# Zhen-Dong/HAWQ

Measured on NVIDIA H100. Metric: images/sec ResNet-50 W8A8 & W4A4 @batch128, 1/2/4/8xH100; % int-TC roofline, higher is better.
Workload: dtype int8

## Files before the change

### hawq_b200/csrc/api.cu

```cuda
#include <cmath>
#include <cstdarg>
#include <cstdio>
#include <cstring>

#include <cstdlib>

#include "conv_igemm.cuh"
#include "elementwise.cuh"
#include "stem.cuh"

using namespace hawq;

struct hawq_handle {
  int device;
  int sm_count;
  int32_t* status;
};

static thread_local char g_err[512] = "";
static long long g_kernel_count[8] = {0, 0, 0, 0, 0, 0, 0, 0};

static int fail(int code, const char* fmt, ...) {
  va_list ap;
  va_start(ap, fmt);
  vsnprintf(g_err, sizeof(g_err), fmt, ap);
  va_end(ap);
  return code;
}

#define CUDA_TRY(expr)                                                                         \
  do {                                                                                         \
    cudaError_t _e = (expr);                                                                   \
    if (_e != cudaSuccess) return fail(HAWQ_ERR_CUDA, "%s: %s", #expr, cudaGetErrorString(_e)); \
  } while (0)

static int launch_check(const char* what) {
  cudaError_t e = cudaGetLastError();
  if (e != cudaSuccess) return fail(HAWQ_ERR_CUDA, "%s launch: %s", what, cudaGetErrorString(e));
  return HAWQ_OK;
}

static int grid_for(long long work_items, int sm_count) {
  long long blocks = (work_items + 255) / 256;
  const long long cap = (long long)sm_count * 16;
  if (blocks > cap) blocks = cap;
  if (blocks < 1) blocks = 1;
  return (int)blocks;
}

template <int BN, bool A4, int FAM, bool DUAL>
static int set_conv_attr1() {
  CUDA_TRY(cudaFuncSetAttribute(conv_igemm_kernel<BN, A4, FAM, DUAL>, cudaFuncAttributeMaxDynamicSharedMemorySize,
                                ConvSmem<BN, A4, DUAL>::TOTAL));
  CUDA_TRY(cudaFuncSetAttribute(conv_igemm_kernel<BN, A4, FAM, DUAL>, cudaFuncAttributePreferredSharedMemoryCarveout,
                                cudaSharedmemCarveoutMaxShared));
  return HAWQ_OK;
}
template <int BN, bool A4>
static int set_conv_attr() {
  int rc;
  if ((rc = set_conv_attr1<BN, A4, FAM_REQUANT, false>()) || (rc = set_conv_attr1<BN, A4, FAM_RESIDUAL, false>()) ||
      (rc = set_conv_attr1<BN, A4, FAM_STORE, false>()))
    return rc;
  return HAWQ_OK;
}

static dim3 conv_grid(long long M, int Cout, int BN) { return dim3((unsigned)((M + CONV_BM - 1) / CONV_BM * (Cout / BN)), 1, 1); }

template <int BN, bool A4>
static void launch_conv(const ConvParams& p, cudaStream_t s) {
  const int smem = ConvSmem<BN, A4, false>::TOTAL;
  const dim3 grid = conv_grid(p.M, p.Cout, BN);
  if (p.mode == HAWQ_EPI_REQUANT) conv_igemm_kernel<BN, A4, FAM_REQUANT, false><<<grid, CONV_THREADS, smem, s>>>(p);
  else if (p.mode == HAWQ_EPI_RESIDUAL) conv_igemm_kernel<BN, A4, FAM_RESIDUAL, false><<<grid, CONV_THREADS, smem, s>>>(p);
  else conv_igemm_kernel<BN, A4, FAM_STORE, false><<<grid, CONV_THREADS, smem, s>>>(p);
}
template <bool A4>
static void launch_conv_dual(const ConvParams& p, cudaStream_t s) {
  conv_igemm_kernel<64, A4, FAM_RESIDUAL, true><<<conv_grid(p.M, p.Cout, 64), CONV_THREADS, ConvSmem<64, A4, true>::TOTAL, s>>>(p);
}

extern "C" {

int hawq_abi_version(void) { return HAWQ_ABI_VERSION; }
const char* hawq_last_error(void) { return g_err; }

int hawq_create(int device, hawq_handle** out) {
  if (!out) return fail(HAWQ_ERR_BAD_ARG, "hawq_create: out is null");
  CUDA_TRY(cudaSetDevice(device));
  cudaDeviceProp prop;
  CUDA_TRY(cudaGetDeviceProperties(&prop, device));
  if (prop.major != 9 || prop.minor != 0)
    return fail(HAWQ_ERR_UNSUPPORTED, "hawq_create: device sm_%d%d is not Hopper sm_90 (the library is built for sm_90a)", prop.major, prop.minor);
  hawq_handle* h = new hawq_handle();
  h->device = device;
  h->sm_count = prop.multiProcessorCount;
  h->status = nullptr;
  CUDA_TRY(cudaMalloc(&h->status, sizeof(int32_t)));
  CUDA_TRY(cudaMemset(h->status, 0, sizeof(int32_t)));
  int rc;
  CUDA_TRY(cudaFuncSetAttribute(linear_dp4a_kernel, cudaFuncAttributeMaxDynamicSharedMemorySize, linear_smem_bytes(LIN_MAX_K)));
  if ((rc = set_conv_attr<128, false>()) || (rc = set_conv_attr<64, false>()) || (rc = set_conv_attr<128, true>()) ||
      (rc = set_conv_attr<64, true>()) || (rc = set_conv_attr1<64, false, FAM_RESIDUAL, true>()) ||
      (rc = set_conv_attr1<64, true, FAM_RESIDUAL, true>()))
    return rc;
  *out = h;
  return HAWQ_OK;
}

int hawq_destroy(hawq_handle* h) {
  if (!h) return HAWQ_OK;
  cudaFree(h->status);
  delete h;
  return HAWQ_OK;
}

int hawq_sm_count(const hawq_handle* h) { return h ? h->sm_count : 0; }

int hawq_reset_status(hawq_handle* h, void* stream) {
  if (!h) return fail(HAWQ_ERR_BAD_ARG, "null handle");
  CUDA_TRY(cudaMemsetAsync(h->status, 0, sizeof(int32_t), (cudaStream_t)stream));
  return HAWQ_OK;
}

int hawq_get_status(hawq_handle* h, void* stream, int32_t* host_flags) {
  if (!h || !host_flags) return fail(HAWQ_ERR_BAD_ARG, "null argument");
  CUDA_TRY(cudaMemcpyAsync(host_flags, h->status, sizeof(int32_t), cudaMemcpyDeviceToHost, (cudaStream_t)stream));
  CUDA_TRY(cudaStreamSynchronize((cudaStream_t)stream));
  return HAWQ_OK;
}

int hawq_copy_status(hawq_handle* h, int32_t* dst, void* stream) {
  if (!h || !dst) return fail(HAWQ_ERR_BAD_ARG, "null argument");
  CUDA_TRY(cudaMemcpyAsync(dst, h->status, sizeof(int32_t), cudaMemcpyDeviceToDevice, (cudaStream_t)stream));
  return HAWQ_OK;
}

static void set_bias_window(ConvParams& p, int a_bits) {
// ... 56 lines not shown
        if (!res_chan) return fail(HAWQ_ERR_BAD_ARG, "hawq_conv2d: res_kind 1 needs res_chan");
      } else if (ep->res_kind == 0) {
        if (ep->res_bits != 16 && ep->res_bits != 32) return fail(HAWQ_ERR_BAD_ARG, "hawq_conv2d: res_bits must be 16/32");
        int rc = check_me(ep->res_m, ep->res_e, "hawq_conv2d residual");
        if (rc) return rc;
      } else return fail(HAWQ_ERR_BAD_ARG, "hawq_conv2d: res_kind must be 0/1");
      if (ep->y_bits != 0 && ep->y_bits != 16 && ep->y_bits != 32) return fail(HAWQ_ERR_BAD_ARG, "hawq_conv2d: y_bits must be 0/16/32");
      if (ep->y_bits == 16 && !ep->relu) return fail(HAWQ_ERR_BAD_ARG, "hawq_conv2d: uint16 residual stream requires relu");
      if (ep->y_bits && !out) return fail(HAWQ_ERR_BAD_ARG, "hawq_conv2d: y_bits set but out is null");
      if (ep->low_bits != 0 && ep->low_bits != 4 && ep->low_bits != 8) return fail(HAWQ_ERR_BAD_ARG, "hawq_conv2d: low_bits must be 0/4/8");
      if (ep->low_bits) {
        if (!out_low) return fail(HAWQ_ERR_BAD_ARG, "hawq_conv2d: low_bits set but out_low is null");
        int rc = check_me(ep->low_m, ep->low_e, "hawq_conv2d low-bit copy");
        if (rc) return rc;
      }
      if (!ep->y_bits && !ep->low_bits) return fail(HAWQ_ERR_BAD_ARG, "hawq_conv2d: RESIDUAL with no output");
      break;
    case HAWQ_EPI_RAW_I32:
      if (!out) return fail(HAWQ_ERR_BAD_ARG, "hawq_conv2d: RAW_I32 needs out");
      break;
    case HAWQ_EPI_DEQUANT_F32:
      if (!out || !fscale) return fail(HAWQ_ERR_BAD_ARG, "hawq_conv2d: DEQUANT_F32 needs out and fscale");
      if (ep->cout_store < 1 || ep->cout_store > d->Cout) return fail(HAWQ_ERR_BAD_ARG, "hawq_conv2d: bad cout_store");
      break;
    default:
      return fail(HAWQ_ERR_BAD_ARG, "hawq_conv2d: unknown epilogue mode %d", ep->mode);
  }

  const bool bn128 = (d->Cout % 128 == 0);
  if ((M + CONV_BM - 1) / CONV_BM * (d->Cout / (bn128 ? 128 : 64)) > 0x7fffffffll)
    return fail(HAWQ_ERR_UNSUPPORTED, "hawq_conv2d: more than 2^31 - 1 output tiles");
  ++g_kernel_count[0];
  cudaStream_t s = (cudaStream_t)stream;
  if (d->a_bits == 8) {
    if (bn128) launch_conv<128, false>(p, s);
    else launch_conv<64, false>(p, s);
  } else {
    if (bn128) launch_conv<128, true>(p, s);
    else launch_conv<64, true>(p, s);
  }
  return launch_check("conv_igemm");
}

int hawq_conv2d_dual(hawq_handle* h, const hawq_conv_desc* d, const hawq_epilogue_desc* ep, const void* x, const int8_t* w,
                     const hawq_chan* chan, const hawq_conv_desc* d2, const void* x2, const int8_t* w2, const hawq_chan* chan2,
                     void* out, void* out_low, void* stream) {
  if (!h || !d || !ep || !x || !w || !chan || !d2 || !x2 || !w2 || !chan2 || !out) return fail(HAWQ_ERR_BAD_ARG, "hawq_conv2d_dual: null argument");
  if (d->kh != 1 || d->kw != 1 || d->stride != 1 || d->pad != 0 || d2->kh != 1 || d2->kw != 1 || d2->pad != 0 || d2->stride < 1)
    return fail(HAWQ_ERR_UNSUPPORTED, "hawq_conv2d_dual: both convolutions must be 1x1 without padding (main stride 1)");
  if (d->N < 1 || d->H < 1 || d->W < 1 || d2->H < 1 || d2->W < 1) return fail(HAWQ_ERR_BAD_ARG, "hawq_conv2d_dual: bad geometry");
  if ((d->a_bits != 8 && d->a_bits != 4) || d2->a_bits != d->a_bits) return fail(HAWQ_ERR_UNSUPPORTED, "hawq_conv2d_dual: a_bits must be equal and 4 or 8");
  if (d->Cin % 64 || d2->Cin % 64 || d->Cout % 64 || d2->Cout != d->Cout) return fail(HAWQ_ERR_UNSUPPORTED, "hawq_conv2d_dual: channel counts must be multiples of 64 and Cout equal");
  if (d2->N != d->N || (d2->H - 1) / d2->stride + 1 != d->H || (d2->W - 1) / d2->stride + 1 != d->W)
    return fail(HAWQ_ERR_BAD_ARG, "hawq_conv2d_dual: the two convolutions have different output grids");
  if (d->w_layout != 1 || d2->w_layout != 1) return fail(HAWQ_ERR_UNSUPPORTED, "hawq_conv2d_dual: weights must carry the re-tiled copy (w_layout 1)");
  if (ep->mode != HAWQ_EPI_RESIDUAL || !ep->relu || ep->y_bits != 16) return fail(HAWQ_ERR_UNSUPPORTED, "hawq_conv2d_dual: RESIDUAL + relu + uint16 stream only");
  if (ep->low_bits != 0 && ep->low_bits != 4 && ep->low_bits != 8) return fail(HAWQ_ERR_BAD_ARG, "hawq_conv2d_dual: low_bits must be 0/4/8");
  if (ep->low_bits) {
    if (!out_low) return fail(HAWQ_ERR_BAD_ARG, "hawq_conv2d_dual: low_bits set but out_low is null");
    int rc = check_me(ep->low_m, ep->low_e, "hawq_conv2d_dual low-bit copy");
    if (rc) return rc;
    if (!dyadic_is_fast(ep->low_m, ep->low_e)) return fail(HAWQ_ERR_UNSUPPORTED, "hawq_conv2d_dual: low-bit ratio outside the fast range");
  }
  const bool ratios_one = (ep->flags & HAWQ_EP_RATIOS_LE_ONE) != 0;
  const bool ratios_wide = !ratios_one && (ep->flags & HAWQ_EP_RATIOS_LE_2P20) != 0;
  if (!ratios_one && !ratios_wide) return fail(HAWQ_ERR_UNSUPPORTED, "hawq_conv2d_dual: needs a ratio-range promise (flags)");
// ... 244 lines not shown
```

### hawq_b200/csrc/conv_igemm.cuh

```cuda
#pragma once
#include <type_traits>

#include "common.cuh"
#include "wgmma.cuh"

namespace hawq {

struct ConvParams {
  const uint8_t* x;
  const int8_t* w;
  const hawq_chan* chan;
  const void* res;
  const hawq_chan* res_chan;
  const float* fscale;
  void* out;
  void* out_low;
  int32_t* status;
  int N, H, W, Cin, Cout, KH, KW, stride, pad, Ho, Wo, M, K;
  int cin_chunks;
  int x_pix_bytes;
  int mode, relu, out_bits, lo, hi;
  int res_kind, res_bits;
  uint32_t res_m;
  int res_e;
  int y_bits, low_bits;
  uint32_t low_m;
  int low_e, low_lo, low_hi;
  int cout_store;
  int scalar_over_one;
  int scalar_unchecked;
  int check_ovf;
  int bias_lo, bias_hi;
  const uint8_t* x2;
  const int8_t* w2;
  int H2, W2, stride2, cin_chunks2, x2_pix_bytes;
};

constexpr int CONV_BM = 128;
constexpr int CONV_STAGES = 4;
constexpr int CONV_THREADS = 256;

template <int BN, bool A4, bool DUAL>
struct ConvSmem {
  static constexpr int A_ROW = A4 ? 32 : 64;
  static constexpr int A_STAGE = CONV_BM * A_ROW;
  static constexpr int B_STAGE = BN * 64;
  static constexpr int PIPE = CONV_STAGES * (A_STAGE + B_STAGE);
  static constexpr int OUT_PITCH = BN + 16;
  static constexpr int OUT_STAGE = CONV_BM * OUT_PITCH;
  static constexpr int RES16 = CONV_BM * (BN * 2 + 16);
  static constexpr int RES32 = CONV_BM * (BN * 4 + 32);
  static constexpr int RES16_OFF = PIPE;
  static constexpr int RES32_OFF = DUAL ? PIPE : OUT_STAGE;
  static constexpr int Y_OFF = OUT_STAGE;
  static constexpr int MAIN = DUAL ? PIPE + RES32 : (PIPE + RES16 > RES32_OFF + RES32 ? PIPE + RES16 : RES32_OFF + RES32);
  static constexpr int CHAN_OFF = MAIN;
  static constexpr int M_OFF = CHAN_OFF + BN * (int)sizeof(hawq_chan);
  static constexpr int M1_OFF = M_OFF + BN * 8;
  static constexpr int RC_OFF = M1_OFF + BN * 8;
  static constexpr int CB_OFF = RC_OFF + BN * (int)sizeof(hawq_chan);
  static constexpr int TOTAL = CB_OFF + BN * 8;
  static_assert(OUT_STAGE <= PIPE && (!DUAL || Y_OFF + RES16 <= PIPE), "the epilogue staging tiles must fit in the freed ring");
  static_assert(2 * (TOTAL + 1024) <= 228 * 1024, "two CTAs per SM must fit in shared memory");
};

template <int ROW_BYTES>
__device__ __forceinline__ int swz(int row, int ch) {
  if constexpr (ROW_BYTES == 64) return row * 64 + ((ch ^ ((row >> 1) & 3)) << 4);
  else return row * 32 + ((ch ^ ((row >> 2) & 1)) << 4);
}

constexpr int FAM_REQUANT = 0, FAM_RESIDUAL = 1, FAM_STORE = 2;

template <bool CLAMPED>
struct RqFp64 {
  bool checked;
  bool ovf = false;
  static constexpr double kMagic = 6755399441055744.0;
  __device__ static double acc_bias(int32_t acc, double cb, int32_t) {
    const double d = __hiloint2double(0x43300000, acc ^ 0x80000000) - cb;
    return CLAMPED ? fmin(fmax(d, -2147483648.0), 2147483647.0) : d;
  }
  __device__ static double of_i32(int32_t v) {
    return __hiloint2double(0x43300000, v ^ 0x80000000) - 4503601774854144.0;
  }
  __device__ static double of_u16(uint32_t u) { return __hiloint2double(0x43300000, (int)u) - 4503599627370496.0; }
  __device__ int32_t term(double d, double M, uint32_t, int32_t, bool count) {
    const double t = __fma_rn(d, M, kMagic);
    if (checked && count) {
      const double q = t - kMagic;
      ovf |= q > 2147483647.0 || q < -2147483648.0;
    }
    return __double2loint(t);
  }
};
struct RqExact {
  bool checked;
  bool ovf = false;
  __device__ static int32_t acc_bias(int32_t acc, double, int32_t bias) { return sat_add(acc, bias); }
  __device__ static int32_t of_i32(int32_t v) { return v; }
  __device__ static int32_t of_u16(uint32_t u) { return (int32_t)u; }
  __device__ int32_t term(int32_t v, double, uint32_t m, int32_t e, bool count) {
    const long long q = rhe_requant64(v, m, e);
    if (checked && count) ovf |= q > 2147483647ll || q < -2147483648ll;
    return sat_i32(q);
  }
};

struct ConvGeom {
  const uint8_t* x;
  const int8_t* w;
  int H, W, stride, pad, KH, KW, cin_chunks, x_pix_bytes, K;
};

template <int BN, bool A4, int FAM, bool DUAL>
__global__ void __launch_bounds__(CONV_THREADS, 2) conv_igemm_kernel(const ConvParams p) {
  using S = ConvSmem<BN, A4, DUAL>;
  constexpr int BM = CONV_BM, STAGES = CONV_STAGES;
  constexpr int A_ROW = S::A_ROW;
  constexpr int A_CH = A_ROW / 16;
  constexpr int A_ROWS_PER_PASS = CONV_THREADS / A_CH;
  constexpr int A_PASSES = BM / A_ROWS_PER_PASS;
  constexpr int B_PASSES = BN / 64;
  constexpr int NT = BN / 8;
  constexpr int NACC = BN / 2;

  extern __shared__ __align__(1024) uint8_t smem[];
  uint8_t* sA = smem;
  uint8_t* sB = smem + STAGES * S::A_STAGE;
  hawq_chan* sChan = reinterpret_cast<hawq_chan*>(smem + S::CHAN_OFF);
  double* sM = reinterpret_cast<double*>(smem + S::M_OFF);
  double* sM1 = reinterpret_cast<double*>(smem + S::M1_OFF);
  hawq_chan* sResChan = reinterpret_cast<hawq_chan*>(smem + S::RC_OFF);
  double* sCb = reinterpret_cast<double*>(smem + S::CB_OFF);

  const int tid = threadIdx.x;
  const int lane = tid & 31, warp = tid >> 5;
  const int wg = warp >> 2;
  const int g = lane >> 2, t = lane & 3;
  const int nblk = p.Cout / BN;
  const int m0 = (int)(blockIdx.x / nblk) * BM;
  const int n0 = (int)(blockIdx.x % nblk) * BN;

  int over_one = p.scalar_over_one;
  int unchecked = p.scalar_unchecked;
  int bias_out = 0;
  if (tid < BN) {
    const hawq_chan c = p.chan[n0 + tid];
    sChan[tid] = c;
    sM[tid] = dyadic_to_double(c.m, c.e);
    sCb[tid] = 4503601774854144.0 - (double)c.bias;
    bias_out = c.bias < p.bias_lo || c.bias > p.bias_hi;
    over_one |= !dyadic_is_fast(c.m, c.e);
    unchecked |= !dyadic_is_wide(c.m, c.e);
    if (FAM == FAM_RESIDUAL && p.res_kind == 1) {
      const hawq_chan rc = p.res_chan[n0 + tid];
      sResChan[tid] = rc;
      sM1[tid] = dyadic_to_double(rc.m, rc.e);
      over_one |= !dyadic_is_fast(rc.m, rc.e);
      unchecked |= !dyadic_is_wide(rc.m, rc.e);
    }
  }
  const bool ratio_over_one = __syncthreads_or(over_one) != 0;
  const bool ratio_unchecked = __syncthreads_or(unchecked) != 0;
  const bool clamped = __syncthreads_or(bias_out) != 0;
  const bool fp64 = !ratio_over_one || (FAM == FAM_RESIDUAL && p.check_ovf && !ratio_unchecked);

  int32_t acc[NACC];

  const int res_es = (FAM == FAM_RESIDUAL) ? ((p.res_kind == 1 || p.res_bits == 32) ? 4 : 2) : 0;
  const int res_pitch = BN * res_es + 8 * res_es;
  uint8_t* sRes = smem + (res_es == 2 ? S::RES16_OFF : S::RES32_OFF);

  auto load_res = [&]() {
    if constexpr (FAM == FAM_RESIDUAL) {
      const int cpr = BN * res_es / 16;
      const uint8_t* gres = reinterpret_cast<const uint8_t*>(p.res);
      for (int id = tid; id < BM * cpr; id += CONV_THREADS) {
        const int row = id / cpr, j = id - row * cpr;
        const bool v = m0 + row < p.M;
        const uint8_t* src = v ? gres + ((size_t)(m0 + row) * p.Cout + n0) * res_es + j * 16 : gres;
        cp_async_16(smem_u32(sRes + row * res_pitch + j * 16), src, v ? 16 : 0);
      }
    }
  };
  const bool prefetch_res = !DUAL && res_es == 2;

  auto gemm = [&](const ConvGeom& gm, bool with_res) {
#pragma unroll
    for (int i = 0; i < NACC; ++i) acc[i] = 0;
    const int a_ch = tid % A_CH;
    int a_hi0[A_PASSES], a_wi0[A_PASSES], a_pix[A_PASSES];
    bool a_ok[A_PASSES];
#pragma unroll
    for (int i = 0; i < A_PASSES; ++i) {
      const int row = tid / A_CH + i * A_ROWS_PER_PASS;
      const int m = m0 + row;
      a_ok[i] = m < p.M;
      const int mm = a_ok[i] ? m : 0;
// ... 48 lines not shown
      cp_async_commit();

      const int stage = kt % STAGES;
      const uint32_t a_base = smem_u32(sA + stage * S::A_STAGE);
      const uint32_t b_base = smem_u32(sB + stage * S::B_STAGE);
#pragma unroll
      for (int ks = 0; ks < 2; ++ks) {
        const uint64_t bdesc = wgmma_desc_sw64(b_base + ks * 32);
        if constexpr (!A4) {
          wgmma_fence();
          wgmma_ss<BN>(acc, wgmma_desc_sw64(a_base + wg * 64 * A_ROW + ks * 32), bdesc);
        } else {
          uint32_t r0, r1;
          const int row = warp * 16 + (lane & 7) + ((lane >> 3) & 1) * 8;
          ldmatrix_x2(r0, r1, a_base + swz<32>(row, ks));
          const uint32_t af[4] = {r0 & 0x0F0F0F0Fu, r1 & 0x0F0F0F0Fu, (r0 >> 4) & 0x0F0F0F0Fu, (r1 >> 4) & 0x0F0F0F0Fu};
          wgmma_fence();
          wgmma_rs<BN>(acc, af, bdesc);
        }
      }
      wgmma_commit();
      wgmma_wait_all();
      fence_operands(acc);
    }
    cp_async_wait<0>();
    __syncthreads();
  };

  if constexpr (DUAL) {
    gemm(ConvGeom{p.x2, p.w2, p.H2, p.W2, p.stride2, 0, 1, 1, p.cin_chunks2, p.x2_pix_bytes, p.cin_chunks2 * 64}, false);
#pragma unroll
    for (int ni = 0; ni < NT; ++ni) {
      const int col = ni * 8 + 2 * t;
      const int b0 = sResChan[col].bias, b1 = sResChan[col + 1].bias;
#pragma unroll
      for (int hf = 0; hf < 2; ++hf) {
        const int row = warp * 16 + hf * 8 + g;
        *reinterpret_cast<int2*>(sRes + row * res_pitch + col * 4) =
            make_int2(sat_add(acc[ni * 4 + hf * 2], b0), sat_add(acc[ni * 4 + hf * 2 + 1], b1));
      }
    }
  }
  gemm(ConvGeom{p.x, p.w, p.H, p.W, p.stride, p.pad, p.KH, p.KW, p.cin_chunks, p.x_pix_bytes, p.K}, prefetch_res);

  if (!DUAL && res_es == 4) {
    load_res();
    cp_async_commit();
    cp_async_wait<0>();
    __syncthreads();
  }
  const bool y_staged = DUAL || (res_es != 0 && p.y_bits == res_es * 8);
  const int y_es = p.y_bits / 8;
  const int y_pitch = BN * y_es + 8 * y_es;
  uint8_t* sY = DUAL ? smem + S::Y_OFF : sRes;

  uint8_t* sOut = smem;
  const bool stage_low = (FAM == FAM_REQUANT && p.out_bits <= 8) || (FAM == FAM_RESIDUAL && p.low_bits != 0);
  const int stage_bits = (FAM == FAM_REQUANT) ? p.out_bits : p.low_bits;

  auto put_low = [&](int row, int col, int q0, int q1) {
    *reinterpret_cast<uint16_t*>(sOut + row * S::OUT_PITCH + col) = (uint16_t)__byte_perm(q0, q1, 0x0040);
  };
  auto put_y = [&](int row, int col, bool ok, int y0, int y1, int& ymax) {
    if (p.y_bits == 16 && ok) ymax = max(ymax, max(y0, y1));
    if (!y_staged && !ok) return;
    uint8_t* dst = y_staged ? sY + row * y_pitch + col * y_es
                            : reinterpret_cast<uint8_t*>(p.out) + ((size_t)(m0 + row) * p.Cout + n0 + col) * y_es;
    if (p.y_bits == 16) *reinterpret_cast<uint32_t*>(dst) = (uint32_t)min(y0, 65535) | ((uint32_t)min(y1, 65535) << 16);
    else if (p.y_bits == 32) *reinterpret_cast<int2*>(dst) = make_int2(y0, y1);
  };

  auto epilogue = [&](auto rq, auto low_out) {
    if constexpr (FAM == FAM_REQUANT) {
      const int lo = p.relu ? min(max(p.lo, 0), p.hi) : p.lo;
#pragma unroll
      for (int ni = 0; ni < NT; ++ni) {
        const int col = ni * 8 + 2 * t;
        const int4 c0 = *reinterpret_cast<const int4*>(&sChan[col]);
        const int4 c1 = *reinterpret_cast<const int4*>(&sChan[col + 1]);
        const double2 M = *reinterpret_cast<const double2*>(&sM[col]);
        const double2 Cb = *reinterpret_cast<const double2*>(&sCb[col]);
#pragma unroll
        for (int hf = 0; hf < 2; ++hf) {
          const int row = warp * 16 + hf * 8 + g;
          const int q0 = clampi(rq.term(rq.acc_bias(acc[ni * 4 + hf * 2], Cb.x, c0.x), M.x, c0.y, c0.z, false), lo, p.hi);
          const int q1 = clampi(rq.term(rq.acc_bias(acc[ni * 4 + hf * 2 + 1], Cb.y, c1.x), M.y, c1.y, c1.z, false), lo, p.hi);
          if constexpr (decltype(low_out)::value) {
            put_low(row, col, q0, q1);
          } else if (m0 + row < p.M) {
            uint8_t* dst = reinterpret_cast<uint8_t*>(p.out) + ((size_t)(m0 + row) * p.Cout + n0 + col) * (p.out_bits / 8);
            if (p.out_bits == 16) *reinterpret_cast<uint32_t*>(dst) = (uint32_t)(q0 & 0xFFFF) | ((uint32_t)q1 << 16);
            else *reinterpret_cast<int2*>(dst) = make_int2(q0, q1);
          }
        }
      }
    } else {
      const double res_M = dyadic_to_double(p.res_m, p.res_e), low_M = dyadic_to_double(p.low_m, p.low_e);
      const int relu_floor = p.relu ? 0 : (int)0x80000000;
      int ymax = 0;
#pragma unroll
      for (int ni = 0; ni < NT; ++ni) {
        const int col = ni * 8 + 2 * t;
        const int4 c0 = *reinterpret_cast<const int4*>(&sChan[col]);
        const int4 c1 = *reinterpret_cast<const int4*>(&sChan[col + 1]);
        const double2 M = *reinterpret_cast<const double2*>(&sM[col]);
        const double2 Cb = *reinterpret_cast<const double2*>(&sCb[col]);
        double2 M1 = make_double2(res_M, res_M);
        uint2 m1 = make_uint2(p.res_m, p.res_m);
        int2 e1 = make_int2(p.res_e, p.res_e);
        if (p.res_kind == 1) {
          M1 = *reinterpret_cast<const double2*>(&sM1[col]);
          m1 = make_uint2(sResChan[col].m, sResChan[col + 1].m);
          e1 = make_int2(sResChan[col].e, sResChan[col + 1].e);
        }
#pragma unroll
        for (int hf = 0; hf < 2; ++hf) {
          const int row = warp * 16 + hf * 8 + g;
          const bool ok = m0 + row < p.M;
          const uint8_t* rptr = sRes + row * res_pitch + col * res_es;
          decltype(rq.of_i32(0)) r0, r1;
          if (res_es == 2) {
            const uint32_t pr = *reinterpret_cast<const uint32_t*>(rptr);
            r0 = rq.of_u16(pr & 0xFFFFu);
            r1 = rq.of_u16(pr >> 16);
          } else {
            const int2 pr = *reinterpret_cast<const int2*>(rptr);
            r0 = rq.of_i32(pr.x);
            r1 = rq.of_i32(pr.y);
          }
          const auto v0 = rq.acc_bias(acc[ni * 4 + hf * 2 + 0], Cb.x, c0.x);
          const auto v1 = rq.acc_bias(acc[ni * 4 + hf * 2 + 1], Cb.y, c1.x);
          const int y0 = max(sat_add(rq.term(r0, M1.x, m1.x, e1.x, ok), rq.term(v0, M.x, c0.y, c0.z, ok)), relu_floor);
          const int y1 = max(sat_add(rq.term(r1, M1.y, m1.y, e1.y, ok), rq.term(v1, M.y, c1.y, c1.z, ok)), relu_floor);
          put_y(row, col, ok, y0, y1, ymax);
          if (p.low_bits != 0)
            put_low(row, col, clampi(rq.term(rq.of_i32(y0), low_M, p.low_m, p.low_e, false), p.low_lo, p.low_hi),
                    clampi(rq.term(rq.of_i32(y1), low_M, p.low_m, p.low_e, false), p.low_lo, p.low_hi));
        }
      }
      if (ymax > 65535) atomicOr(p.status, HAWQ_FLAG_RESIDUAL_OVERFLOW);
      if (rq.ovf) atomicOr(p.status, HAWQ_FLAG_REQUANT_OVERFLOW);
    }
  };

  if constexpr (FAM == FAM_STORE) {
#pragma unroll
    for (int ni = 0; ni < NT; ++ni) {
      const int col = ni * 8 + 2 * t;
      const int b0 = sChan[col].bias, b1 = sChan[col + 1].bias;
#pragma unroll
      for (int hf = 0; hf < 2; ++hf) {
        const int m = m0 + warp * 16 + hf * 8 + g;
        if (m >= p.M) continue;
        const int32_t v0 = sat_add(acc[ni * 4 + hf * 2 + 0], b0), v1 = sat_add(acc[ni * 4 + hf * 2 + 1], b1);
        if (p.mode == HAWQ_EPI_RAW_I32) {
          *reinterpret_cast<int2*>(reinterpret_cast<int32_t*>(p.out) + (size_t)m * p.Cout + n0 + col) = make_int2(v0, v1);
        } else {
          float* o = reinterpret_cast<float*>(p.out) + (size_t)m * p.cout_store;
          const int c = n0 + col;
          if (c < p.cout_store) o[c] = __fmul_rn((float)v0, p.fscale[c]);
          if (c + 1 < p.cout_store) o[c + 1] = __fmul_rn((float)v1, p.fscale[c + 1]);
        }
      }
    }
  } else {
    auto run = [&](auto low_out) {
      if (!fp64) epilogue(RqExact{FAM == FAM_RESIDUAL && p.check_ovf}, low_out);
      else if (clamped) epilogue(RqFp64<true>{FAM == FAM_RESIDUAL && ratio_over_one}, low_out);
      else epilogue(RqFp64<false>{FAM == FAM_RESIDUAL && ratio_over_one}, low_out);
    };
    if (FAM == FAM_REQUANT && p.out_bits <= 8) run(std::true_type{});
    else run(std::false_type{});
  }

  if (y_staged || stage_low) __syncthreads();
  if (y_staged) {
    const int cpr = BN * y_es / 16;
    uint8_t* gy = reinterpret_cast<uint8_t*>(p.out);
    for (int id = tid; id < BM * cpr; id += CONV_THREADS) {
      const int row = id / cpr, j = id - row * cpr;
      if (m0 + row < p.M)
        *reinterpret_cast<int4*>(gy + ((size_t)(m0 + row) * p.Cout + n0) * y_es + j * 16) =
            *reinterpret_cast<const int4*>(sY + row * y_pitch + j * 16);
    }
  }
  if (stage_low) {
    uint8_t* gout = reinterpret_cast<uint8_t*>(FAM == FAM_REQUANT ? p.out : p.out_low);
    if (stage_bits == 8) {
      constexpr int CPR = BN / 16;
      for (int id = tid; id < BM * CPR; id += CONV_THREADS) {
        const int row = id / CPR, j = id % CPR;
        if (m0 + row < p.M) {
          const int4 v = *reinterpret_cast<const int4*>(sOut + row * S::OUT_PITCH + j * 16);
          *reinterpret_cast<int4*>(gout + (size_t)(m0 + row) * p.Cout + n0 + j * 16) = v;
        }
      }
    } else {
      constexpr int CPR = BN / 32;
      for (int id = tid; id < BM * CPR; id += CONV_THREADS) {
        const int row = id / CPR, j = id % CPR;
        if (m0 + row < p.M) {
          const uint4 a = *reinterpret_cast<const uint4*>(sOut + row * S::OUT_PITCH + j * 32);
          const uint4 b = *reinterpret_cast<const uint4*>(sOut + row * S::OUT_PITCH + j * 32 + 16);
          uint4 o;
          o.x = pack_nibbles8(a.x, a.y);
          o.y = pack_nibbles8(a.z, a.w);
          o.z = pack_nibbles8(b.x, b.y);
          o.w = pack_nibbles8(b.z, b.w);
          *reinterpret_cast<uint4*>(gout + (((size_t)(m0 + row) * p.Cout + n0 + j * 32) >> 1)) = o;
        }
      }
    }
  }
}

}
```

Baseline: 24140.

## Add persistent weight-resident tail kernel for 1x1 residual convolutions

Adds a persistent conv_tail_kernel for stride-1, unpadded 1x1 int8 convolutions with a 16-bit residual epilogue. Each CTA loads its full 128-column weight slice into shared memory once, then loops over row tiles, prefetching activations and the residual tile through a 2-3 stage cp.async ring. This removes repeated weight reloads and per-tile launch and prologue cost for the small-K conv+residual layers. The change also moves the channel setup and residual epilogue out of the main kernel into shared helpers. The new kernel runs one CTA per SM with a large shared-memory footprint, and the grid is capped at roughly the SM count, which may reduce latency hiding.

```diff
diff --git a/hawq_b200/csrc/api.cu b/hawq_b200/csrc/api.cu
--- a/hawq_b200/csrc/api.cu
+++ b/hawq_b200/csrc/api.cu
@@ -6,6 +6,7 @@
 #include <cstdlib>
 
 #include "conv_igemm.cuh"
+#include "conv_tail.cuh"
 #include "elementwise.cuh"
 #include "stem.cuh"
 
@@ -62,6 +63,13 @@
   if ((rc = set_conv_attr1<BN, A4, FAM_REQUANT, false>()) || (rc = set_conv_attr1<BN, A4, FAM_RESIDUAL, false>()) ||
       (rc = set_conv_attr1<BN, A4, FAM_STORE, false>()))
     return rc;
+  return HAWQ_OK;
+}
+
+template <int NBUF, int K_MAX>
+static int set_tail_attr() {
+  CUDA_TRY(cudaFuncSetAttribute(conv_tail_kernel<NBUF>, cudaFuncAttributeMaxDynamicSharedMemorySize, TailSmem<NBUF>::total(K_MAX)));
+  CUDA_TRY(cudaFuncSetAttribute(conv_tail_kernel<NBUF>, cudaFuncAttributePreferredSharedMemoryCarveout, cudaSharedmemCarveoutMaxShared));
   return HAWQ_OK;
 }
 
@@ -104,6 +112,7 @@
       (rc = set_conv_attr<64, true>()) || (rc = set_conv_attr1<64, false, FAM_RESIDUAL, true>()) ||
       (rc = set_conv_attr1<64, true, FAM_RESIDUAL, true>()))
     return rc;
+  if ((rc = set_tail_attr<2, TAIL_MAX_K>()) || (rc = set_tail_attr<3, 128>())) return rc;
   *out = h;
   return HAWQ_OK;
 }
@@ -226,6 +235,17 @@
     return fail(HAWQ_ERR_UNSUPPORTED, "hawq_conv2d: more than 2^31 - 1 output tiles");
   ++g_kernel_count[0];
   cudaStream_t s = (cudaStream_t)stream;
+  if (ep->mode == HAWQ_EPI_RESIDUAL && ep->res_kind == 0 && ep->res_bits == 16 && ep->y_bits == 16 && d->kh == 1 && d->kw == 1 &&
+      d->stride == 1 && d->pad == 0 && d->a_bits == 8 && d->Cin <= TAIL_MAX_K && d->Cout % TAIL_BN == 0) {
+    const int nblk = d->Cout / TAIL_BN;
+    const long long row_tiles = (M + CONV_BM - 1) / CONV_BM;
+    const int slots = h->sm_count / nblk > 1 ? h->sm_count / nblk : 1;
+    const int R = (int)(row_tiles < slots ? row_tiles : slots);
+    ++g_kernel_count[5];
+    if (tail_nbuf(p.K) == 3) conv_tail_kernel<3><<<nblk * R, CONV_THREADS, TailSmem<3>::total(p.K), s>>>(p, R);
+    else conv_tail_kernel<2><<<nblk * R, CONV_THREADS, TailSmem<2>::total(p.K), s>>>(p, R);
+    return launch_check("conv_tail");
+  }
   if (d->a_bits == 8) {
     if (bn128) launch_conv<128, false>(p, s);
     else launch_conv<64, false>(p, s);
diff --git a/hawq_b200/csrc/conv_igemm.cuh b/hawq_b200/csrc/conv_igemm.cuh
--- a/hawq_b200/csrc/conv_igemm.cuh
+++ b/hawq_b200/csrc/conv_igemm.cuh
@@ -55,11 +55,7 @@
   static constexpr int Y_OFF = OUT_STAGE;
   static constexpr int MAIN = DUAL ? PIPE + RES32 : (PIPE + RES16 > RES32_OFF + RES32 ? PIPE + RES16 : RES32_OFF + RES32);
   static constexpr int CHAN_OFF = MAIN;
-  static constexpr int M_OFF = CHAN_OFF + BN * (int)sizeof(hawq_chan);
-  static constexpr int M1_OFF = M_OFF + BN * 8;
-  static constexpr int RC_OFF = M1_OFF + BN * 8;
-  static constexpr int CB_OFF = RC_OFF + BN * (int)sizeof(hawq_chan);
-  static constexpr int TOTAL = CB_OFF + BN * 8;
+  static constexpr int TOTAL = CHAN_OFF + BN * (2 * (int)sizeof(hawq_chan) + 3 * 8);
   static_assert(OUT_STAGE <= PIPE && (!DUAL || Y_OFF + RES16 <= PIPE), "the epilogue staging tiles must fit in the freed ring");
   static_assert(2 * (TOTAL + 1024) <= 228 * 1024, "two CTAs per SM must fit in shared memory");
 };
@@ -106,6 +102,191 @@
     return sat_i32(q);
   }
 };
+
+
+template <int BN>
+struct ChanArrays {
+  static constexpr int BYTES = BN * (2 * (int)sizeof(hawq_chan) + 3 * 8);
+  hawq_chan* chan;
+  double* M;
+  double* M1;
+  hawq_chan* res_chan;
+  double* Cb;
+  __device__ explicit ChanArrays(uint8_t* base)
+      : chan(reinterpret_cast<hawq_chan*>(base)),
+        M(reinterpret_cast<double*>(base + BN * (int)sizeof(hawq_chan))),
+        M1(reinterpret_cast<double*>(base + BN * (int)sizeof(hawq_chan) + BN * 8)),
+        res_chan(reinterpret_cast<hawq_chan*>(base + BN * (int)sizeof(hawq_chan) + 2 * BN * 8)),
+        Cb(reinterpret_cast<double*>(base + 2 * BN * (int)sizeof(hawq_chan) + 2 * BN * 8)) {}
+};
+
+struct RqPolicy {
+  bool fp64;
+  bool clamped;
+  bool over_one;
+};
+
+template <int BN, int FAM>
+__device__ __forceinline__ RqPolicy conv_channels(const ConvParams& p, int n0, const ChanArrays<BN>& cs) {
+  const int tid = threadIdx.x;
+  int over_one = p.scalar_over_one;
+  int unchecked = p.scalar_unchecked;
+  int bias_out = 0;
+  if (tid < BN) {
+    const hawq_chan c = p.chan[n0 + tid];
+    cs.chan[tid] = c;
+    cs.M[tid] = dyadic_to_double(c.m, c.e);
+    cs.Cb[tid] = 4503601774854144.0 - (double)c.bias;
+    bias_out = c.bias < p.bias_lo || c.bias > p.bias_hi;
+    over_one |= !dyadic_is_fast(c.m, c.e);
+    unchecked |= !dyadic_is_wide(c.m, c.e);
+    if (FAM == FAM_RESIDUAL && p.res_kind == 1) {
+      const hawq_chan rc = p.res_chan[n0 + tid];
+      cs.res_chan[tid] = rc;
+      cs.M1[tid] = dyadic_to_double(rc.m, rc.e);
+      over_one |= !dyadic_is_fast(rc.m, rc.e);
+      unchecked |= !dyadic_is_wide(rc.m, rc.e);
+    }
+  }
+  RqPolicy pol;
+  pol.over_one = __syncthreads_or(over_one) != 0;
+  const bool ratio_unchecked = __syncthreads_or(unchecked) != 0;
+  pol.clamped = __syncthreads_or(bias_out) != 0;
+  pol.fp64 = !pol.over_one || (FAM == FAM_RESIDUAL && p.check_ovf && !ratio_unchecked);
+  return pol;
+}
+
+template <int FAM, class F>
+__device__ __forceinline__ void with_rq(const RqPolicy& pol, const ConvParams& p, F&& f) {
+  if (!pol.fp64) f(RqExact{FAM == FAM_RESIDUAL && p.check_ovf});
+  else if (pol.clamped) f(RqFp64<true>{FAM == FAM_RESIDUAL && pol.over_one});
+  else f(RqFp64<false>{FAM == FAM_RESIDUAL && pol.over_one});
+}
+
+template <int BN>
+__device__ __forceinline__ void put_low(uint8_t* sOut, int row, int col, int q0, int q1) {
+  *reinterpret_cast<uint16_t*>(sOut + row * (BN + 16) + col) = (uint16_t)__byte_perm(q0, q1, 0x0040);
+}
+
+struct ResidualIO {
+  const uint8_t* res;
+  int res_pitch, res_es;
+  uint8_t* y;
+  int y_pitch;
+  bool y_staged;
+  uint8_t* low;
+};
+
+template <int BN, int TAIL = 0, class Rq>
+__device__ __forceinline__ void residual_epilogue(Rq& rq, const int32_t (&acc)[BN / 2], const ConvParams& p, const ChanArrays<BN>& cs,
+                                                  const ResidualIO& io, int m0, int n0, int& ymax) {
+  constexpr int NT = BN / 8;
+  const int lane = threadIdx.x & 31, warp = threadIdx.x >> 5;
+  const int g = lane >> 2, t = lane & 3;
+  const int y_bits = TAIL ? 16 : p.y_bits;
+  const bool y_staged = TAIL ? true : io.y_staged;
+  const int res_es = TAIL ? 2 : io.res_es;
+  const bool res_chan = TAIL ? false : p.res_kind == 1;
+  const bool low = TAIL ? TAIL == 2 : p.low_bits != 0;
+  const int y_es = y_bits / 8;
+  auto put_y = [&](int row, int col, bool ok, int y0, int y1) {
+    if (y_bits == 16 && ok) ymax = max(ymax, max(y0, y1));
+    if (!y_staged && !ok) return;
+    uint8_t* dst = y_staged ? io.y + row * io.y_pitch + col * y_es
+                            : reinterpret_cast<uint8_t*>(p.out) + ((size_t)(m0 + row) * p.Cout + n0 + col) * y_es;
+    if (y_bits == 16) *reinterpret_cast<uint32_t*>(dst) = (uint32_t)min(y0, 65535) | ((uint32_t)min(y1, 65535) << 16);
+    else if (y_bits == 32) *reinterpret_cast<int2*>(dst) = make_int2(y0, y1);
+  };
+  const double res_M = dyadic_to_double(p.res_m, p.res_e), low_M = dyadic_to_double(p.low_m, p.low_e);
+  const int relu_floor = p.relu ? 0 : (int)0x80000000;
+#pragma unroll
+  for (int ni = 0; ni < NT; ++ni) {
+    const int col = ni * 8 + 2 * t;
+    const int4 c0 = *reinterpret_cast<const int4*>(&cs.chan[col]);
+    const int4 c1 = *reinterpret_cast<const int4*>(&cs.chan[col + 1]);
+    const double2 M = *reinterpret_cast<const double2*>(&cs.M[col]);
+    const double2 Cb = *reinterpret_cast<const double2*>(&cs.Cb[col]);
+    double2 M1 = make_double2(res_M, res_M);
+    uint2 m1 = make_uint2(p.res_m, p.res_m);
+    int2 e1 = make_int2(p.res_e, p.res_e);
+    if (res_chan) {
+      M1 = *reinterpret_cast<const double2*>(&cs.M1[col]);
+      m1 = make_uint2(cs.res_chan[col].m, cs.res_chan[col + 1].m);
+      e1 = make_int2(cs.res_chan[col].e, cs.res_chan[col + 1].e);
+    }
+#pragma unroll
+    for (int hf = 0; hf < 2; ++hf) {
+      const int row = warp * 16 + hf * 8 + g;
+      const bool ok = m0 + row < p.M;
+      const uint8_t* rptr = io.res + row * io.res_pitch + col * res_es;
+      decltype(rq.of_i32(0)) r0, r1;
+      if (res_es == 2) {
+        const uint32_t pr = *reinterpret_cast<const uint32_t*>(rptr);
+        r0 = rq.of_u16(pr & 0xFFFFu);
+        r1 = rq.of_u16(pr >> 16);
+      } else {
+        const int2 pr = *reinterpret_cast<const int2*>(rptr);
+        r0 = rq.of_i32(pr.x);
+        r1 = rq.of_i32(pr.y);
+      }
+      const auto v0 = rq.acc_bias(acc[ni * 4 + hf * 2 + 0], Cb.x, c0.x);
+      const auto v1 = rq.acc_bias(acc[ni * 4 + hf * 2 + 1], Cb.y, c1.x);
+      const int y0 = max(sat_add(rq.term(r0, M1.x, m1.x, e1.x, ok), rq.term(v0, M.x, c0.y, c0.z, ok)), relu_floor);
+      const int y1 = max(sat_add(rq.term(r1, M1.y, m1.y, e1.y, ok), rq.term(v1, M.y, c1.y, c1.z, ok)), relu_floor);
+      put_y(row, col, ok, y0, y1);
+      if (low)
+        put_low<BN>(io.low, row, col, clampi(rq.term(rq.of_i32(y0), low_M, p.low_m, p.low_e, false), p.low_lo, p.low_hi),
+                    clampi(rq.term(rq.of_i32(y1), low_M, p.low_m, p.low_e, false), p.low_lo, p.low_hi));
+    }
+  }
+}
+
+__device__ __forceinline__ void residual_flags(int32_t* status, int ymax, bool ovf) {
+  if (ymax > 65535) atomicOr(status, HAWQ_FLAG_RESIDUAL_OVERFLOW);
+  if (ovf) atomicOr(status, HAWQ_FLAG_REQUANT_OVERFLOW);
+}
+
+template <int BN>
+__device__ __forceinline__ void store_y_tile(const ConvParams& p, const uint8_t* sY, int y_pitch, int y_es, int m0, int n0) {
+  const int cpr = BN * y_es / 16;
+  uint8_t* gy = reinterpret_cast<uint8_t*>(p.out);
+  for (int id = threadIdx.x; id < CONV_BM * cpr; id += CONV_THREADS) {
+    const int row = id / cpr, j = id - row * cpr;
+    if (m0 + row < p.M)
+      *reinterpret_cast<int4*>(gy + ((size_t)(m0 + row) * p.Cout + n0) * y_es + j * 16) =
+          *reinterpret_cast<const int4*>(sY + row * y_pitch + j * 16);
+  }
+}
+
+template <int BN>
+__device__ __forceinline__ void store_low_tile(const ConvParams& p, uint8_t* gout, const uint8_t* sOut, int bits, int m0, int n0) {
+  constexpr int OUT_PITCH = BN + 16;
+  if (bits == 8) {
+    constexpr int CPR = BN / 16;
+    for (int id = threadIdx.x; id < CONV_BM * CPR; id += CONV_THREADS) {
+      const int row = id / CPR, j = id % CPR;
+      if (m0 + row < p.M) {
+        const int4 v = *reinterpret_cast<const int4*>(sOut + row * OUT_PITCH + j * 16);
+        *reinterpret_cast<int4*>(gout + (size_t)(m0 + row) * p.Cout + n0 + j * 16) = v;
+      }
+    }
+  } else {
+    constexpr int CPR = BN / 32;
+    for (int id = threadIdx.x; id < CONV_BM * CPR; id += CONV_THREADS) {
+      const int row = id / CPR, j = id % CPR;
+      if (m0 + row < p.M) {
+        const uint4 a = *reinterpret_cast<const uint4*>(sOut + row * OUT_PITCH + j * 32);
+        const uint4 b = *reinterpret_cast<const uint4*>(sOut + row * OUT_PITCH + j * 32 + 16);
+        uint4 o;
+        o.x = pack_nibbles8(a.x, a.y);
+        o.y = pack_nibbles8(a.z, a.w);
+        o.z = pack_nibbles8(b.x, b.y);
+        o.w = pack_nibbles8(b.z, b.w);
+        *reinterpret_cast<uint4*>(gout + (((size_t)(m0 + row) * p.Cout + n0 + j * 32) >> 1)) = o;
+      }
+    }
+  }
+}
 
 struct ConvGeom {
   const uint8_t* x;
@@ -128,11 +309,7 @@
   extern __shared__ __align__(1024) uint8_t smem[];
   uint8_t* sA = smem;
   uint8_t* sB = smem + STAGES * S::A_STAGE;
-  hawq_chan* sChan = reinterpret_cast<hawq_chan*>(smem + S::CHAN_OFF);
-  double* sM = reinterpret_cast<double*>(smem + S::M_OFF);
-  double* sM1 = reinterpret_cast<double*>(smem + S::M1_OFF);
-  hawq_chan* sResChan = reinterpret_cast<hawq_chan*>(smem + S::RC_OFF);
-  double* sCb = reinterpret_cast<double*>(smem + S::CB_OFF);
+  const ChanArrays<BN> cs(smem + S::CHAN_OFF);
 
   const int tid = threadIdx.x;
   const int lane = tid & 31, warp = tid >> 5;
@@ -142,29 +319,7 @@
   const int m0 = (int)(blockIdx.x / nblk) * BM;
   const int n0 = (int)(blockIdx.x % nblk) * BN;
 
-  int over_one = p.scalar_over_one;
-  int unchecked = p.scalar_unchecked;
-  int bias_out = 0;
-  if (tid < BN) {
-    const hawq_chan c = p.chan[n0 + tid];
-    sChan[tid] = c;
-    sM[tid] = dyadic_to_double(c.m, c.e);
-    sCb[tid] = 4503601774854144.0 - (double)c.bias;
-    bias_out = c.bias < p.bias_lo || c.bias > p.bias_hi;
-    over_one |= !dyadic_is_fast(c.m, c.e);
-    unchecked |= !dyadic_is_wide(c.m, c.e);
-    if (FAM == FAM_RESIDUAL && p.res_kind == 1) {
-      const hawq_chan rc = p.res_chan[n0 + tid];
-      sResChan[tid] = rc;
-      sM1[tid] = dyadic_to_double(rc.m, rc.e);
-      over_one |= !dyadic_is_fast(rc.m, rc.e);
-      unchecked |= !dyadic_is_wide(rc.m, rc.e);
-    }
-  }
-  const bool ratio_over_one = __syncthreads_or(over_one) != 0;
-  const bool ratio_unchecked = __syncthreads_or(unchecked) != 0;
-  const bool clamped = __syncthreads_or(bias_out) != 0;
-  const bool fp64 = !ratio_over_one || (FAM == FAM_RESIDUAL && p.check_ovf && !ratio_unchecked);
+  const RqPolicy pol = conv_channels<BN, FAM>(p, n0, cs);
 
   int32_t acc[NACC];
 
@@ -279,7 +434,7 @@
 #pragma unroll
     for (int ni = 0; ni < NT; ++ni) {
       const int col = ni * 8 + 2 * t;
-      const int b0 = sResChan[col].bias, b1 = sResChan[col + 1].bias;
+      const int b0 = cs.res_chan[col].bias, b1 = cs.res_chan[col + 1].bias;
 #pragma unroll
       for (int hf = 0; hf < 2; ++hf) {
         const int row = warp * 16 + hf * 8 + g;
@@ -305,35 +460,23 @@
   const bool stage_low = (FAM == FAM_REQUANT && p.out_bits <= 8) || (FAM == FAM_RESIDUAL && p.low_bits != 0);
   const int stage_bits = (FAM == FAM_REQUANT) ? p.out_bits : p.low_bits;
 
-  auto put_low = [&](int row, int col, int q0, int q1) {
-    *reinterpret_cast<uint16_t*>(sOut + row * S::OUT_PITCH + col) = (uint16_t)__byte_perm(q0, q1, 0x0040);
-  };
-  auto put_y = [&](int row, int col, bool ok, int y0, int y1, int& ymax) {
-    if (p.y_bits == 16 && ok) ymax = max(ymax, max(y0, y1));
-    if (!y_staged && !ok) return;
-    uint8_t* dst = y_staged ? sY + row * y_pitch + col * y_es
-                            : reinterpret_cast<uint8_t*>(p.out) + ((size_t)(m0 + row) * p.Cout + n0 + col) * y_es;
-    if (p.y_bits == 16) *reinterpret_cast<uint32_t*>(dst) = (uint32_t)min(y0, 65535) | ((uint32_t)min(y1, 65535) << 16);
-    else if (p.y_bits == 32) *reinterpret_cast<int2*>(dst) = make_int2(y0, y1);
-  };
-
   auto epilogue = [&](auto rq, auto low_out) {
     if constexpr (FAM == FAM_REQUANT) {
       const int lo = p.relu ? min(max(p.lo, 0), p.hi) : p.lo;
 #pragma unroll
       for (int ni = 0; ni < NT; ++ni) {
         const int col = ni * 8 + 2 * t;
-        const int4 c0 = *reinterpret_cast<const int4*>(&sChan[col]);
-        const int4 c1 = *reinterpret_cast<const int4*>(&sChan[col + 1]);
-        const double2 M = *reinterpret_cast<const double2*>(&sM[col]);
-        const double2 Cb = *reinterpret_cast<const double2*>(&sCb[col]);
+        const int4 c0 = *reinterpret_cast<const int4*>(&cs.chan[col]);
+        const int4 c1 = *reinterpret_cast<const int4*>(&cs.chan[col + 1]);
+        const double2 M = *reinterpret_cast<const double2*>(&cs.M[col]);
+        const double2 Cb = *reinterpret_cast<const double2*>(&cs.Cb[col]);
 #pragma unroll
         for (int hf = 0; hf < 2; ++hf) {
           const int row = warp * 16 + hf * 8 + g;
           const int q0 = clampi(rq.term(rq.acc_bias(acc[ni * 4 + hf * 2], Cb.x, c0.x), M.x, c0.y, c0.z, false), lo, p.hi);
           const int q1 = clampi(rq.term(rq.acc_bias(acc[ni * 4 + hf * 2 + 1], Cb.y, c1.x), M.y, c1.y, c1.z, false), lo, p.hi);
           if constexpr (decltype(low_out)::value) {
-            put_low(row, col, q0, q1);
+            put_low<BN>(sOut, row, col, q0, q1);
           } else if (m0 + row < p.M) {
             uint8_t* dst = reinterpret_cast<uint8_t*>(p.out) + ((size_t)(m0 + row) * p.Cout + n0 + col) * (p.out_bits / 8);
             if (p.out_bits == 16) *reinterpret_cast<uint32_t*>(dst) = (uint32_t)(q0 & 0xFFFF) | ((uint32_t)q1 << 16);
@@ -342,51 +485,9 @@
         }
       }
     } else {
-      const double res_M = dyadic_to_double(p.res_m, p.res_e), low_M = dyadic_to_double(p.low_m, p.low_e);
-      const int relu_floor = p.relu ? 0 : (int)0x80000000;
       int ymax = 0;
-#pragma unroll
-      for (int ni = 0; ni < NT; ++ni) {
-        const int col = ni * 8 + 2 * t;
-        const int4 c0 = *reinterpret_cast<const int4*>(&sChan[col]);
-        const int4 c1 = *reinterpret_cast<const int4*>(&sChan[col + 1]);
-        const double2 M = *reinterpret_cast<const double2*>(&sM[col]);
-        const double2 Cb = *reinterpret_cast<const double2*>(&sCb[col]);
-        double2 M1 = make_double2(res_M, res_M);
-        uint2 m1 = make_uint2(p.res_m, p.res_m);
-        int2 e1 = make_int2(p.res_e, p.res_e);
-        if (p.res_kind == 1) {
-          M1 = *reinterpret_cast<const double2*>(&sM1[col]);
-          m1 = make_uint2(sResChan[col].m, sResChan[col + 1].m);
-          e1 = make_int2(sResChan[col].e, sResChan[col + 1].e);
-        }
-#pragma unroll
-        for (int hf = 0; hf < 2; ++hf) {
-          const int row = warp * 16 + hf * 8 + g;
-          const bool ok = m0 + row < p.M;
-          const uint8_t* rptr = sRes + row * res_pitch + col * res_es;
-          decltype(rq.of_i32(0)) r0, r1;
-          if (res_es == 2) {
-            const uint32_t pr = *reinterpret_cast<const uint32_t*>(rptr);
-            r0 = rq.of_u16(pr & 0xFFFFu);
-            r1 = rq.of_u16(pr >> 16);
-          } else {
-            const int2 pr = *reinterpret_cast<const int2*>(rptr);
-            r0 = rq.of_i32(pr.x);
-            r1 = rq.of_i32(pr.y);
-          }
-          const auto v0 = rq.acc_bias(acc[ni * 4 + hf * 2 + 0], Cb.x, c0.x);
-          const auto v1 = rq.acc_bias(acc[ni * 4 + hf * 2 + 1], Cb.y, c1.x);
-          const int y0 = max(sat_add(rq.term(r0, M1.x, m1.x, e1.x, ok), rq.term(v0, M.x, c0.y, c0.z, ok)), relu_floor);
-          const int y1 = max(sat_add(rq.term(r1, M1.y, m1.y, e1.y, ok), rq.term(v1, M.y, c1.y, c1.z, ok)), relu_floor);
-          put_y(row, col, ok, y0, y1, ymax);
-          if (p.low_bits != 0)
-            put_low(row, col, clampi(rq.term(rq.of_i32(y0), low_M, p.low_m, p.low_e, false), p.low_lo, p.low_hi),
-                    clampi(rq.term(rq.of_i32(y1), low_M, p.low_m, p.low_e, false), p.low_lo, p.low_hi));
-        }
-      }
-      if (ymax > 65535) atomicOr(p.status, HAWQ_FLAG_RESIDUAL_OVERFLOW);
-      if (rq.ovf) atomicOr(p.status, HAWQ_FLAG_REQUANT_OVERFLOW);
+      residual_epilogue<BN>(rq, acc, p, cs, ResidualIO{sRes, res_pitch, res_es, sY, y_pitch, y_staged, sOut}, m0, n0, ymax);
+      residual_flags(p.status, ymax, rq.ovf);
     }
   };
 
@@ -394,7 +495,7 @@
 #pragma unroll
     for (int ni = 0; ni < NT; ++ni) {
       const int col = ni * 8 + 2 * t;
-      const int b0 = sChan[col].bias, b1 = sChan[col + 1].bias;
+      const int b0 = cs.chan[col].bias, b1 = cs.chan[col + 1].bias;
 #pragma unroll
       for (int hf = 0; hf < 2; ++hf) {
         const int m = m0 + warp * 16 + hf * 8 + g;
@@ -411,54 +512,14 @@
       }
     }
   } else {
-    auto run = [&](auto low_out) {
-      if (!fp64) epilogue(RqExact{FAM == FAM_RESIDUAL && p.check_ovf}, low_out);
-      else if (clamped) epilogue(RqFp64<true>{FAM == FAM_RESIDUAL && ratio_over_one}, low_out);
-      else epilogue(RqFp64<false>{FAM == FAM_RESIDUAL && ratio_over_one}, low_out);
-    };
+    auto run = [&](auto low_out) { with_rq<FAM>(pol, p, [&](auto rq) { epilogue(rq, low_out); }); };
     if (FAM == FAM_REQUANT && p.out_bits <= 8) run(std::true_type{});
     else run(std::false_type{});
   }
 
   if (y_staged || stage_low) __syncthreads();
-  if (y_staged) {
-    const int cpr = BN * y_es / 16;
-    uint8_t* gy = reinterpret_cast<uint8_t*>(p.out);
-    for (int id = tid; id < BM * cpr; id += CONV_THREADS) {
-      const int row = id / cpr, j = id - row * cpr;
-      if (m0 + row < p.M)
-        *reinterpret_cast<int4*>(gy + ((size_t)(m0 + row) * p.Cout + n0) * y_es + j * 16) =
-            *reinterpret_cast<const int4*>(sY + row * y_pitch + j * 16);
-    }
-  }
-  if (stage_low) {
-    uint8_t* gout = reinterpret_cast<uint8_t*>(FAM == FAM_REQUANT ? p.out : p.out_low);
-    if (stage_bits == 8) {
-      constexpr int CPR = BN / 16;
-      for (int id = tid; id < BM * CPR; id += CONV_THREADS) {
-        const int row = id / CPR, j = id % CPR;
-        if (m0 + row < p.M) {
-          const int4 v = *reinterpret_cast<const int4*>(sOut + row * S::OUT_PITCH + j * 16);
-          *reinterpret_cast<int4*>(gout + (size_t)(m0 + row) * p.Cout + n0 + j * 16) = v;
-        }
-      }
-    } else {
-      constexpr int CPR = BN / 32;
-      for (int id = tid; id < BM * CPR; id += CONV_THREADS) {
-        const int row = id / CPR, j = id % CPR;
-        if (m0 + row < p.M) {
-          const uint4 a = *reinterpret_cast<const uint4*>(sOut + row * S::OUT_PITCH + j * 32);
-          const uint4 b = *reinterpret_cast<const uint4*>(sOut + row * S::OUT_PITCH + j * 32 + 16);
-          uint4 o;
-          o.x = pack_nibbles8(a.x, a.y);
-          o.y = pack_nibbles8(a.z, a.w);
-          o.z = pack_nibbles8(b.x, b.y);
-          o.w = pack_nibbles8(b.z, b.w);
-          *reinterpret_cast<uint4*>(gout + (((size_t)(m0 + row) * p.Cout + n0 + j * 32) >> 1)) = o;
-        }
-      }
-    }
-  }
-}
-
-}
+  if (y_staged) store_y_tile<BN>(p, sY, y_pitch, y_es, m0, n0);
+  if (stage_low) store_low_tile<BN>(p, reinterpret_cast<uint8_t*>(FAM == FAM_REQUANT ? p.out : p.out_low), sOut, stage_bits, m0, n0);
+}
+
+}
diff --git a/hawq_b200/csrc/conv_tail.cuh b/hawq_b200/csrc/conv_tail.cuh
--- /dev/null
+++ b/hawq_b200/csrc/conv_tail.cuh
@@ -0,0 +1,112 @@
+#pragma once
+#include "conv_igemm.cuh"
+
+namespace hawq {
+
+constexpr int TAIL_BN = 128;
+constexpr int TAIL_MAX_K = 256;
+__host__ __device__ constexpr int tail_nbuf(int K) { return K <= 128 ? 3 : 2; }
+
+template <int NBUF>
+struct TailSmem {
+  static constexpr int RES_PITCH = TAIL_BN * 2 + 16;
+  static constexpr int RES16 = CONV_BM * RES_PITCH;
+  static constexpr int OUT_STAGE = CONV_BM * (TAIL_BN + 16);
+  __host__ __device__ static constexpr int buf(int K) { return CONV_BM * K + RES16; }
+  __host__ __device__ static constexpr int buf_off(int K, int b) { return TAIL_BN * K + b * buf(K); }
+  __host__ __device__ static constexpr int low_off(int K) { return buf_off(K, NBUF); }
+  __host__ __device__ static constexpr int chan_off(int K) { return low_off(K) + OUT_STAGE; }
+  __host__ __device__ static constexpr int total(int K) { return chan_off(K) + ChanArrays<TAIL_BN>::BYTES; }
+};
+static_assert(TailSmem<2>::RES16 % 512 == 0, "A tiles must stay 512-B aligned");
+static_assert(TailSmem<tail_nbuf(TAIL_MAX_K)>::total(TAIL_MAX_K) <= 227 * 1024 && TailSmem<tail_nbuf(128)>::total(128) <= 227 * 1024,
+              "one CTA per SM must fit in shared memory");
+
+template <int NBUF>
+__global__ void __launch_bounds__(CONV_THREADS, 1) conv_tail_kernel(const ConvParams p, int R) {
+  using TailSmem = hawq::TailSmem<NBUF>;
+  constexpr int BM = CONV_BM, BN = TAIL_BN;
+  extern __shared__ __align__(1024) uint8_t smem[];
+  const int tid = threadIdx.x;
+  const int wg = tid >> 7;
+  const int K = p.K, CPR = K / 16;
+  const int nblk = p.Cout / BN;
+  const int n0 = (int)(blockIdx.x % nblk) * BN;
+  const int first = (int)(blockIdx.x / nblk);
+  const int ntiles = ((p.M + BM - 1) / BM - first + R - 1) / R;
+  const ChanArrays<BN> cs(smem + TailSmem::chan_off(K));
+  uint8_t* sLow = smem + TailSmem::low_off(K);
+
+  for (int id = tid; id < BN * CPR; id += CONV_THREADS) {
+    const int row = id / CPR, c = id - row * CPR;
+    cp_async_16(smem_u32(smem + (c >> 2) * (BN * 64) + swz<64>(row, c & 3)), p.w + (size_t)(n0 + row) * K + c * 16, 16);
+  }
+  auto load_tile = [&](int j, int b) {
+    const int m0 = (first + j * R) * BM;
+    uint8_t* sA = smem + TailSmem::buf_off(K, b);
+    uint8_t* sRes = sA + BM * K;
+    for (int id = tid; id < BM * CPR; id += CONV_THREADS) {
+      const int row = id / CPR, c = id - row * CPR;
+      const bool v = m0 + row < p.M;
+      const uint8_t* src = v ? p.x + (size_t)(m0 + row) * K + c * 16 : p.x;
+      cp_async_16(smem_u32(sA + (c >> 2) * (BM * 64) + swz<64>(row, c & 3)), src, v ? 16 : 0);
+    }
+    const uint8_t* gres = reinterpret_cast<const uint8_t*>(p.res);
+    for (int id = tid; id < BM * (BN / 8); id += CONV_THREADS) {
+      const int row = id / (BN / 8), c = id % (BN / 8);
+      const bool v = m0 + row < p.M;
+      const uint8_t* src = v ? gres + ((size_t)(m0 + row) * p.Cout + n0) * 2 + c * 16 : gres;
+      cp_async_16(smem_u32(sRes + row * TailSmem::RES_PITCH + c * 16), src, v ? 16 : 0);
+    }
+  };
+#pragma unroll
+  for (int s = 0; s < NBUF - 1; ++s) {
+    if (s < ntiles) load_tile(s, s);
+    cp_async_commit();
+  }
+
+  const RqPolicy pol = conv_channels<BN, FAM_RESIDUAL>(p, n0, cs);
+  const uint32_t w_base = smem_u32(smem);
+  int ymax = 0;
+  bool ovf = false;
+  int32_t acc[BN / 2];
+
+  for (int j = 0; j < ntiles; ++j) {
+    const int b = j % NBUF;
+    uint8_t* sA = smem + TailSmem::buf_off(K, b);
+    uint8_t* sRes = sA + BM * K;
+    cp_async_wait<NBUF - 2>();
+    fence_proxy_async_smem();
+    __syncthreads();
+    if (j + NBUF - 1 < ntiles) load_tile(j + NBUF - 1, (j + NBUF - 1) % NBUF);
+    cp_async_commit();
+
+#pragma unroll
+    for (int i = 0; i < BN / 2; ++i) acc[i] = 0;
+    const uint32_t a_base = smem_u32(sA) + wg * 64 * 64;
+    for (int kb = 0; kb < K / 64; ++kb) {
+#pragma unroll
+      for (int ks = 0; ks < 2; ++ks) {
+        wgmma_fence();
+        wgmma_ss<BN>(acc, wgmma_desc_sw64(a_base + kb * (BM * 64) + ks * 32), wgmma_desc_sw64(w_base + kb * (BN * 64) + ks * 32));
+      }
+    }
+    wgmma_commit();
+    wgmma_wait_all();
+    fence_operands(acc);
+
+    const int m0 = (first + j * R) * BM;
+    const ResidualIO io{sRes, TailSmem::RES_PITCH, 2, sRes, TailSmem::RES_PITCH, true, sLow};
+    with_rq<FAM_RESIDUAL>(pol, p, [&](auto rq) {
+      if (p.low_bits != 0) residual_epilogue<BN, 2>(rq, acc, p, cs, io, m0, n0, ymax);
+      else residual_epilogue<BN, 1>(rq, acc, p, cs, io, m0, n0, ymax);
+      ovf |= rq.ovf;
+    });
+    __syncthreads();
+    store_y_tile<BN>(p, sRes, TailSmem::RES_PITCH, 2, m0, n0);
+    if (p.low_bits != 0) store_low_tile<BN>(p, reinterpret_cast<uint8_t*>(p.out_low), sLow, p.low_bits, m0, n0);
+  }
+  residual_flags(p.status, ymax, ovf);
+}
+
+}
```

Measured after the change: 25890, median of 6. +7.3%, better.
